# xuekt98/BBDM

Hardware: NVIDIA H100
Metric: denoising-steps/sec (UNet fwd) at 256^2 pixel-BBDM (higher is better)
Workload: dtype bf16x3 (split-bf16 tensor-core products, fp32 accumulate: fp32-class)

## Files before the change

bbdm_b200/csrc/conv_umma.cu:

```cuda
#include "tc_common.cuh"
#include <stdlib.h>

namespace bbdm {

constexpr int UM_BM = 128;
constexpr int UM_BK = 64;
constexpr int UM_THREADS = 384;
constexpr int UM_PRODUCER_REGS = 40, UM_CONSUMER_REGS = 232;
static_assert(128 * UM_PRODUCER_REGS + 256 * UM_CONSUMER_REGS <= 65536, "conv_umma: register split");
constexpr int UM_SLICES = 4;

struct ConvParams {
  int B, H, W, Cout;
  int TW, TH, TB, tiles_w, tiles_h, tiles_b, n_tiles;
  int kb_per_tap;
  int K1;
  int K2;
  int taps;
  int up2;
  int origin;
  int w_per_image;
  int kb_per_chunk;
  const float* bias; const float* bias2;
  const float* residual; int res_mode;
  float* out; __nv_bfloat16* out_hi; __nv_bfloat16* out_lo;
  int out_nchw_c;
  float* stats;
  unsigned long long* fault;
};

template <int BN>
struct UmmaCfg {
  static constexpr uint32_t A_BYTES = UM_BM * UM_BK * 2;
  static constexpr uint32_t W_BYTES = BN * UM_BK * 2;
  static constexpr uint32_t STAGE3 = 2 * A_BYTES + 2 * W_BYTES;
  static constexpr uint32_t STAGE1 = A_BYTES + W_BYTES;
  static constexpr uint32_t SMEM_BUDGET = 200 * 1024;
  static constexpr int STAGES3 = (SMEM_BUDGET / STAGE3) > 6 ? 6 : (SMEM_BUDGET / STAGE3);
  static constexpr int STAGES1 = (SMEM_BUDGET / STAGE1) > 8 ? 8 : (SMEM_BUDGET / STAGE1);
};

template <int BN, bool F16>
__device__ __forceinline__ void conv_mma(float* d, uint64_t da, uint64_t db) {
  if (F16) {
    if (BN == 128) wgmma_n128_f16<0>(d, da, db, 1u); else wgmma_n64_f16<0>(d, da, db, 1u);
  } else {
    if (BN == 128) wgmma_n128_bf16<0>(d, da, db, 1u); else wgmma_n64_bf16<0>(d, da, db, 1u);
  }
}

struct EpiTile {
  int nb, tw, th, tb, phase;
  int bb[2], hh[2], ww[2];
  bool valid[2];
  int64_t pix[2];
};

__device__ __forceinline__ EpiTile epi_tile(const ConvParams& p, int tile, int n_blocks, int warp, int lane) {
  EpiTile e;
  e.nb = tile % n_blocks;
  int mt = tile / n_blocks;
  e.phase = 0;
  if (p.up2) { e.phase = mt & 3; mt >>= 2; }
  e.tw = mt % p.tiles_w; mt /= p.tiles_w;
  e.th = mt % p.tiles_h;
  e.tb = mt / p.tiles_h;
  const int OH = p.up2 ? 2 * p.H : p.H, OW = p.up2 ? 2 * p.W : p.W;
#pragma unroll
  for (int ri = 0; ri < 2; ++ri) {
    const int row = 16 * warp + (lane >> 2) + 8 * ri;
    const int ws = e.tw * p.TW + row % p.TW;
    const int hs = e.th * p.TH + (row / p.TW) % p.TH;
    e.bb[ri] = e.tb * p.TB + row / (p.TW * p.TH);
    e.valid[ri] = ws < p.W && hs < p.H && e.bb[ri] < p.B;
    e.hh[ri] = p.up2 ? 2 * hs + (e.phase >> 1) : hs;
    e.ww[ri] = p.up2 ? 2 * ws + (e.phase & 1) : ws;
    e.pix[ri] = ((int64_t)e.bb[ri] * OH + e.hh[ri]) * OW + e.ww[ri];
  }
  return e;
}

template <int BN>
__device__ __forceinline__ void epi_slice(const ConvParams& p, const float* racc, EpiTile e, int s, int warp,
                                          int lane, float (*stats_s)[BN][2]) {
  constexpr int JS = BN / 8 / UM_SLICES;
  asm volatile("" : "+r"(e.nb), "+r"(e.bb[0]), "+r"(e.bb[1]), "+r"(e.hh[0]), "+r"(e.hh[1]), "+r"(e.ww[0]),
               "+r"(e.ww[1]), "+l"(e.pix[0]), "+l"(e.pix[1]));
  const int OH = p.up2 ? 2 * p.H : p.H, OW = p.up2 ? 2 * p.W : p.W;
  const int n0 = e.nb * BN + 2 * (lane & 3);
  float2 v[2][JS];
#pragma unroll
  for (int ri = 0; ri < 2; ++ri) {
#pragma unroll
    for (int j = 0; j < JS; ++j) {
      const int jj = JS * s + j;
      const int nc = n0 + 8 * jj;
      v[ri][j] = make_float2(racc[4 * jj + 2 * ri], racc[4 * jj + 2 * ri + 1]);
      if (p.bias) { const float2 b = *reinterpret_cast<const float2*>(p.bias + nc); v[ri][j].x += b.x; v[ri][j].y += b.y; }
      if (p.bias2) { const float2 b = *reinterpret_cast<const float2*>(p.bias2 + nc); v[ri][j].x += b.x; v[ri][j].y += b.y; }
    }
  }
  if (p.res_mode == BBDM_RES_SAME || p.res_mode == BBDM_RES_UP2) {
#pragma unroll
    for (int ri = 0; ri < 2; ++ri) {
      if (!e.valid[ri]) continue;
      const int64_t rpix = p.res_mode == BBDM_RES_SAME
                               ? e.pix[ri]
                               : ((int64_t)e.bb[ri] * (OH >> 1) + (e.hh[ri] >> 1)) * (OW >> 1) + (e.ww[ri] >> 1);
      const float* rp = p.residual + rpix * p.Cout + n0 + 8 * JS * s;
#pragma unroll
      for (int j = 0; j < JS; ++j) {
        const float2 t = *reinterpret_cast<const float2*>(rp + 8 * j);
        v[ri][j].x += t.x; v[ri][j].y += t.y;
      }
    }
  } else if (p.res_mode == BBDM_RES_DOWN2) {
    const int64_t W2 = (int64_t)OW * 2;
#pragma unroll
    for (int ri = 0; ri < 2; ++ri) {
      if (!e.valid[ri]) continue;
      const float* rp0 = p.residual + (((int64_t)e.bb[ri] * OH * 2 + e.hh[ri] * 2) * W2 + e.ww[ri] * 2) * p.Cout +
                         n0 + 8 * JS * s;
#pragma unroll
      for (int j = 0; j < JS; ++j) {
        const float* rp = rp0 + 8 * j;
        const float2 t0 = *reinterpret_cast<const float2*>(rp), t1 = *reinterpret_cast<const float2*>(rp + p.Cout);
        const float2 t2 = *reinterpret_cast<const float2*>(rp + W2 * p.Cout);
        const float2 t3 = *reinterpret_cast<const float2*>(rp + (W2 + 1) * p.Cout);
        v[ri][j].x += 0.25f * (((t0.x + t1.x) + t2.x) + t3.x);
        v[ri][j].y += 0.25f * (((t0.y + t1.y) + t2.y) + t3.y);
      }
    }
  }
  float ssum[2 * JS], ssq[2 * JS];
#pragma unroll
  for (int j = 0; j < 2 * JS; ++j) { ssum[j] = 0.f; ssq[j] = 0.f; }
#pragma unroll
  for (int ri = 0; ri < 2; ++ri) {
    if (!e.valid[ri]) continue;
    const int bb = e.bb[ri], hh = e.hh[ri], ww = e.ww[ri];
    const int64_t pix = e.pix[ri];
#pragma unroll
    for (int j = 0; j < JS; ++j) {
      const int nc = n0 + 8 * (JS * s + j);
      const float2 w = v[ri][j];
      if (p.out_nchw_c > 0) {
        if (nc < p.out_nchw_c) p.out[(((int64_t)bb * p.out_nchw_c + nc) * OH + hh) * OW + ww] = w.x;
        if (nc + 1 < p.out_nchw_c) p.out[(((int64_t)bb * p.out_nchw_c + nc + 1) * OH + hh) * OW + ww] = w.y;
      } else if (p.out) {
        *reinterpret_cast<float2*>(p.out + pix * p.Cout + nc) = w;
      }
      if (p.out_hi) {
        uint32_t h, l;
        split2x(w.x, w.y, h, l);
        *reinterpret_cast<uint32_t*>(p.out_hi + pix * p.Cout + nc) = h;
        *reinterpret_cast<uint32_t*>(p.out_lo + pix * p.Cout + nc) = l;
      }
      ssum[2 * j] += w.x; ssq[2 * j] += w.x * w.x;
      ssum[2 * j + 1] += w.y; ssq[2 * j + 1] += w.y * w.y;
    }
  }
  if (p.stats) {
#pragma unroll
    for (int j = 0; j < 2 * JS; ++j) {
#pragma unroll
      for (int off = 4; off < 32; off <<= 1) {
        ssum[j] += __shfl_xor_sync(0xffffffffu, ssum[j], off);
        ssq[j] += __shfl_xor_sync(0xffffffffu, ssq[j], off);
      }
    }
    if (lane < 4) {
#pragma unroll
      for (int j = 0; j < 2 * JS; ++j) {
        const int c = 8 * (JS * s + (j >> 1)) + 2 * lane + (j & 1);
        stats_s[warp][c][0] = ssum[j];
        stats_s[warp][c][1] = ssq[j];
      }
    }
  }
}

template <int BN>
__device__ __forceinline__ void epi_stats_out(const ConvParams& p, const EpiTile& e, float (*stats_s)[BN][2]) {
  if (!p.stats) return;
  asm volatile("bar.sync 1, 256;" ::: "memory");
  const int64_t tile_lin =
      (((int64_t)e.tb * p.tiles_w * p.tiles_h + e.th * p.tiles_w + e.tw) * (p.up2 ? 4 : 1) + e.phase) * 4;
  int i0 = threadIdx.x;
  asm volatile("" : "+r"(i0));
  for (int i = i0; i < 4 * BN; i += 256) {
    const int q = i / BN, c = i % BN;
    const float s = stats_s[2 * q][c][0] + stats_s[2 * q + 1][c][0];
    const float sq = stats_s[2 * q][c][1] + stats_s[2 * q + 1][c][1];
    *reinterpret_cast<float2*>(p.stats + ((tile_lin + q) * p.Cout + e.nb * BN + c) * 2) = make_float2(s, sq);
  }
  asm volatile("bar.sync 1, 256;" ::: "memory");
}

template <int BN>
__device__ __forceinline__ void epi_slices(const ConvParams& p, const float* racc, const EpiTile& e, int s_begin,
                                           int s_end, int warp, int lane, float (*stats_s)[BN][2]) {
#pragma unroll
  for (int s = 0; s < UM_SLICES; ++s)
    if (s >= s_begin && s < s_end) epi_slice<BN>(p, racc, e, s, warp, lane, stats_s);
}

template <int BN, int PASSES, bool F16>
__global__ void __launch_bounds__(UM_THREADS, 1)
conv_umma_kernel(const __grid_constant__ CUtensorMap map_a_hi, const __grid_constant__ CUtensorMap map_a_lo,
                 const __grid_constant__ CUtensorMap map_w_hi, const __grid_constant__ CUtensorMap map_w_lo,
                 const __grid_constant__ CUtensorMap map_a2_hi, const __grid_constant__ CUtensorMap map_a2_lo,
                 const __grid_constant__ CUtensorMap map_w2_hi, const __grid_constant__ CUtensorMap map_w2_lo,
                 const ConvParams p) {
  using Cfg = UmmaCfg<BN>;
  constexpr int STAGES = PASSES == 3 ? Cfg::STAGES3 : Cfg::STAGES1;
  constexpr uint32_t STAGE_BYTES = PASSES == 3 ? Cfg::STAGE3 : Cfg::STAGE1;
  constexpr uint32_t OFF_ALO = Cfg::A_BYTES;
  constexpr uint32_t OFF_WHI = PASSES == 3 ? 2 * Cfg::A_BYTES : Cfg::A_BYTES;
  constexpr uint32_t OFF_WLO = OFF_WHI + Cfg::W_BYTES;
  constexpr int NR = BN / 2;
  static_assert(STAGES >= 2, "need at least a double buffer");

  extern __shared__ uint8_t smem_raw[];
  __shared__ __align__(8) uint64_t bars[2 * 8];
  __shared__ int abort_s;
  __shared__ __align__(16) float stats_s[8][BN][2];

  const uint32_t tiles_base = (smem_u32(smem_raw) + 1023u) & ~1023u;
  const int warp = threadIdx.x >> 5, lane = threadIdx.x & 31;
  const uint32_t bar_full = smem_u32(&bars[0]);
  const uint32_t bar_empty = smem_u32(&bars[8]);
  volatile int* abort_flag = &abort_s;

  if (threadIdx.x == 0) {
    abort_s = 0;
    for (int i = 0; i < STAGES; ++i) { mbar_init(bar_full + 8 * i, 1); mbar_init(bar_empty + 8 * i, 8); }
    asm volatile("fence.mbarrier_init.release.cluster;" ::: "memory");
  }
  __syncthreads();

  const int n_blocks = p.Cout / BN;
  const int total_tiles = p.n_tiles * n_blocks * (p.up2 ? 4 : 1);
  const int KB = p.K1 + p.K2;

  if (warp >= 8) {
    setmaxnreg_dec<UM_PRODUCER_REGS>();
    if (warp == 8 && lane == 0) {
      int stage = 0;
      uint32_t phase_bit = 0;
      for (int tile = blockIdx.x; tile < total_tiles; tile += gridDim.x) {
        const int nb = tile % n_blocks;
        int mt = tile / n_blocks;
        int phase = 0;
        if (p.up2) { phase = mt & 3; mt >>= 2; }
        const int tw = mt % p.tiles_w; mt /= p.tiles_w;
        const int th = mt % p.tiles_h;
        const int tb = mt / p.tiles_h;
        const int w0 = tw * p.TW, h0 = th * p.TH, b0 = tb * p.TB, n0 = nb * BN;
        for (int kb = 0; kb < KB; ++kb) {
          mbar_wait(bar_empty + 8 * stage, phase_bit ^ 1, abort_flag, p.fault, 0xE0000000ull | (unsigned)kb);
          const uint32_t sbase = tiles_base + stage * STAGE_BYTES;
          const uint32_t full = bar_full + 8 * stage;
          mbar_expect_tx(full, STAGE_BYTES);
          if (kb < p.K1) {
            const int tap = kb / p.kb_per_tap, cb = kb - tap * p.kb_per_tap;
            int dy = 0, dx = 0, wtap = tap;
            if (p.up2) {
              const int r = tap >> 1, c = tap & 1;
              dy = (phase >> 1) ? r : r - 1;
              dx = (phase & 1) ? c : c - 1;
              wtap = phase * 4 + tap;
            } else if (p.taps == 9) { dy = tap / 3 - 1; dx = tap % 3 - 1; }
            else if (p.taps == 4) { dy = (tap >> 1) + p.origin; dx = (tap & 1) + p.origin; }
            else if (p.w_per_image) wtap = tb;
            tma_load_4d(sbase, &map_a_hi, full, cb * UM_BK, w0 + dx, h0 + dy, b0);
            if (PASSES == 3) tma_load_4d(sbase + OFF_ALO, &map_a_lo, full, cb * UM_BK, w0 + dx, h0 + dy, b0);
            tma_load_3d(sbase + OFF_WHI, &map_w_hi, full, cb * UM_BK, n0, wtap);
            if (PASSES == 3) tma_load_3d(sbase + OFF_WLO, &map_w_lo, full, cb * UM_BK, n0, wtap);
          } else {
            const int cb = kb - p.K1;
            tma_load_4d(sbase, &map_a2_hi, full, cb * UM_BK, w0, h0, b0);
            if (PASSES == 3) tma_load_4d(sbase + OFF_ALO, &map_a2_lo, full, cb * UM_BK, w0, h0, b0);
            tma_load_3d(sbase + OFF_WHI, &map_w2_hi, full, cb * UM_BK, n0, 0);
            if (PASSES == 3) tma_load_3d(sbase + OFF_WLO, &map_w2_lo, full, cb * UM_BK, n0, 0);
          }
          if (++stage == STAGES) { stage = 0; phase_bit ^= 1; }
        }
      }
    }
    return;
  }

  setmaxnreg_inc<UM_CONSUMER_REGS>();
  const int wg = warp >> 2;
  const uint32_t a_off = (uint32_t)wg * 64 * 128;
  int stage = 0;
  uint32_t phase_bit = 0;
  float racc[NR];
  EpiTile pend;
  bool pending = false;
  int slice = 0;
  for (int tile = blockIdx.x; tile < total_tiles; tile += gridDim.x) {
    for (int kb0 = 0; kb0 < KB; kb0 += p.kb_per_chunk) {
      const int kb1 = kb0 + p.kb_per_chunk < KB ? kb0 + p.kb_per_chunk : KB;
      float acc[NR];
#pragma unroll
      for (int j = 0; j < NR; ++j) acc[j] = 0.f;
      int prev = -1;
      for (int kb = kb0; kb < kb1; ++kb) {
        mbar_wait(bar_full + 8 * stage, phase_bit, abort_flag, p.fault, 0xF0000000ull | (unsigned)kb);
        const uint32_t sbase = tiles_base + stage * STAGE_BYTES;
        const uint64_t da_hi = make_sw128_desc(sbase + a_off);
        const uint64_t da_lo = make_sw128_desc(sbase + OFF_ALO + a_off);
        const uint64_t db_hi = make_sw128_desc(sbase + OFF_WHI);
        const uint64_t db_lo = make_sw128_desc(sbase + OFF_WLO);
        wgmma_fence();
#pragma unroll
        for (int k = 0; k < UM_BK / 16; ++k) {
          const uint64_t ko = (uint64_t)(k * 32 >> 4);
          if (PASSES == 3) {
            conv_mma<BN, F16>(acc, da_lo + ko, db_hi + ko);
            conv_mma<BN, F16>(acc, da_hi + ko, db_lo + ko);
          }
          conv_mma<BN, F16>(acc, da_hi + ko, db_hi + ko);
        }
        wgmma_commit();
        wgmma_wait<1>();
        if (prev >= 0 && lane == 0) mbar_arrive(bar_empty + 8 * prev);
        prev = stage;
        if (++stage == STAGES) { stage = 0; phase_bit ^= 1; }
        if (pending) {
          const int s_end = kb + 1 < kb1 ? slice + 1 : UM_SLICES;
          epi_slices<BN>(p, racc, pend, slice, s_end, warp, lane, stats_s);
          slice = s_end;
        }
      }
      if (pending) {
        epi_stats_out<BN>(p, pend, stats_s);
        pending = false;
      }
      wgmma_wait<0>();
      reg_fence<NR>(acc);
      if (lane == 0) mbar_arrive(bar_empty + 8 * prev);
      if (kb0 == 0) {
#pragma unroll
        for (int j = 0; j < NR; ++j) racc[j] = 0.f + acc[j];
      } else {
#pragma unroll
        for (int j = 0; j < NR; ++j) racc[j] += acc[j];
      }
    }
    pend = epi_tile(p, tile, n_blocks, warp, lane);
    pending = true;
    slice = 0;
  }
  if (pending) {
    epi_slices<BN>(p, racc, pend, 0, UM_SLICES, warp, lane, stats_s);
    epi_stats_out<BN>(p, pend, stats_s);
  }
}

static int make_act_map(CUtensorMap* m, const void* ptr, int B, int H, int W, int C, int TW, int TH, int TB,
                        bool f16) {
  EncodeTiledFn enc = get_encode();
  BBDM_REQUIRE(enc != nullptr, "cuTensorMapEncodeTiled entry point not available");
  cuuint64_t dims[4] = {(cuuint64_t)C, (cuuint64_t)W, (cuuint64_t)H, (cuuint64_t)B};
  cuuint64_t strides[3] = {(cuuint64_t)C * 2, (cuuint64_t)W * C * 2, (cuuint64_t)H * W * C * 2};
  cuuint32_t box[4] = {(cuuint32_t)UM_BK, (cuuint32_t)TW, (cuuint32_t)TH, (cuuint32_t)TB};
  cuuint32_t es[4] = {1, 1, 1, 1};
  CUresult r = enc(m, f16 ? CU_TENSOR_MAP_DATA_TYPE_FLOAT16 : CU_TENSOR_MAP_DATA_TYPE_BFLOAT16, 4, const_cast<void*>(ptr), dims, strides, box, es,
                   CU_TENSOR_MAP_INTERLEAVE_NONE, CU_TENSOR_MAP_SWIZZLE_128B, CU_TENSOR_MAP_L2_PROMOTION_L2_256B,
                   CU_TENSOR_MAP_FLOAT_OOB_FILL_NONE);
  BBDM_REQUIRE(r == CUDA_SUCCESS, "cuTensorMapEncodeTiled(activation) failed: %d (B=%d H=%d W=%d C=%d box=%dx%dx%d)",
               (int)r, B, H, W, C, TW, TH, TB);
  return BBDM_OK;
}

static int make_w_map(CUtensorMap* m, const void* ptr, int taps, int Cout, int Cin, int BN, bool f16) {
  EncodeTiledFn enc = get_encode();
  BBDM_REQUIRE(enc != nullptr, "cuTensorMapEncodeTiled entry point not available");
  cuuint64_t dims[3] = {(cuuint64_t)Cin, (cuuint64_t)Cout, (cuuint64_t)taps};
  cuuint64_t strides[2] = {(cuuint64_t)Cin * 2, (cuuint64_t)Cout * Cin * 2};
  cuuint32_t box[3] = {(cuuint32_t)UM_BK, (cuuint32_t)BN, 1};
  cuuint32_t es[3] = {1, 1, 1};
  CUresult r = enc(m, f16 ? CU_TENSOR_MAP_DATA_TYPE_FLOAT16 : CU_TENSOR_MAP_DATA_TYPE_BFLOAT16, 3, const_cast<void*>(ptr), dims, strides, box, es,
                   CU_TENSOR_MAP_INTERLEAVE_NONE, CU_TENSOR_MAP_SWIZZLE_128B, CU_TENSOR_MAP_L2_PROMOTION_L2_256B,
                   CU_TENSOR_MAP_FLOAT_OOB_FILL_NONE);
  BBDM_REQUIRE(r == CUDA_SUCCESS, "cuTensorMapEncodeTiled(weight) failed: %d (taps=%d Cout=%d Cin=%d BN=%d)", (int)r,
               taps, Cout, Cin, BN);
  return BBDM_OK;
}

static int pow2_floor(int x) { int p = 1; while (p * 2 <= x) p *= 2; return p; }
static int pow2_ceil(int x) { int p = 1; while (p < x) p *= 2; return p; }

template <int BN, int PASSES, bool F16>
static int launch_conv(const CUtensorMap* maps, const ConvParams& p, int grid, cudaStream_t s) {
  using Cfg = UmmaCfg<BN>;
  constexpr int STAGES = PASSES == 3 ? Cfg::STAGES3 : Cfg::STAGES1;
  constexpr uint32_t STAGE_BYTES = PASSES == 3 ? Cfg::STAGE3 : Cfg::STAGE1;
  const size_t smem = (size_t)STAGES * STAGE_BYTES + 1024;
  static DeviceOnce configured;
  if (configured.need()) {
    BBDM_CUDA_CHECK(cudaFuncSetAttribute(conv_umma_kernel<BN, PASSES, F16>, cudaFuncAttributeMaxDynamicSharedMemorySize, (int)smem));
    configured.mark();
  }
  conv_umma_kernel<BN, PASSES, F16><<<grid, UM_THREADS, smem, s>>>(maps[0], maps[1], maps[2], maps[3], maps[4], maps[5],
                                                                  maps[6], maps[7], p);
  BBDM_LAUNCH_CHECK();
  return BBDM_OK;
}

}

using namespace bbdm;

static void tile_geometry(int H, int W, int* TW, int* TH, int* TB) {
  *TW = pow2_floor(W) < 16 ? pow2_floor(W) : 16;
  const int th = pow2_ceil(H);
  *TH = th < UM_BM / *TW ? th : UM_BM / *TW;
  *TB = UM_BM / (*TW * *TH);
}

extern "C" int bbdm_conv_umma_geometry(int H, int W, int* TW, int* TH, int* TB, int* rows_per_image) {
  BBDM_REQUIRE(H > 0 && W >= 4, "conv_umma_geometry: need H > 0, W >= 4");
  int tw, th, tb;
  tile_geometry(H, W, &tw, &th, &tb);
  if (TW) *TW = tw;
  if (TH) *TH = th;
  if (TB) *TB = tb;
  if (rows_per_image) *rows_per_image = tb == 1 ? 4 * ((W + tw - 1) / tw) * ((H + th - 1) / th) : 0;
  return BBDM_OK;
}

extern "C" int bbdm_conv_umma(const BbdmConvArgs* a, void* stream) {
  BBDM_REQUIRE(a != nullptr, "conv_umma: null args");
  BBDM_REQUIRE(a->B > 0 && a->H > 0 && a->W > 0, "conv_umma: bad spatial shape");
  BBDM_REQUIRE(a->taps == 1 || a->taps == 9 || a->taps == 4, "conv_umma: taps must be 1, 4 or 9 (got %d)", a->taps);
  BBDM_REQUIRE(!a->upsample2x || (a->taps == 4 && a->Cin2 == 0), "conv_umma: upsample2x needs the 16 phase taps and no fused 1x1");
  BBDM_REQUIRE(a->Cin > 0 && a->Cin % 64 == 0, "conv_umma: Cin %% 64 != 0 (Cin=%d)", a->Cin);
  BBDM_REQUIRE(a->Cout > 0 && a->Cout % 64 == 0, "conv_umma: Cout %% 64 != 0 (Cout=%d)", a->Cout);
  BBDM_REQUIRE(a->Cin2 >= 0 && a->Cin2 % 64 == 0, "conv_umma: Cin2 %% 64 != 0 (Cin2=%d)", a->Cin2);
  BBDM_REQUIRE(a->passes == 1 || a->passes == 3, "conv_umma: passes must be 1 or 3");
  BBDM_REQUIRE(a->a_hi && a->w_hi && (a->passes == 1 || (a->a_lo && a->w_lo)), "conv_umma: missing operand plane");
  if (a->Cin2) BBDM_REQUIRE(a->a2_hi && a->w2_hi && (a->passes == 1 || (a->a2_lo && a->w2_lo)), "conv_umma: missing 1x1 operand plane");
  BBDM_REQUIRE(a->out || (a->out_hi && a->out_lo), "conv_umma: no output");
  BBDM_REQUIRE((a->out_hi == nullptr) == (a->out_lo == nullptr), "conv_umma: out hi/lo must come in pairs");
  BBDM_REQUIRE(a->res_mode >= 0 && a->res_mode <= 3 && (a->res_mode == 0 || a->residual), "conv_umma: bad residual");
  if (a->res_mode == BBDM_RES_UP2 && !a->upsample2x) BBDM_REQUIRE(a->H % 2 == 0 && a->W % 2 == 0, "conv_umma: RES_UP2 needs even H, W");
  BBDM_REQUIRE(a->W >= 4, "conv_umma: W < 4 not supported (use conv_direct)");
  BBDM_REQUIRE(a->window_origin == 0 || a->window_origin == -1, "conv_umma: window_origin must be 0 or -1 (got %d)",
               a->window_origin);
  BBDM_REQUIRE(a->window_origin == 0 || (a->taps == 4 && !a->upsample2x),
               "conv_umma: window_origin -1 needs taps == 4 and no upsample2x");
  const bool wpi = a->weights_per_image != 0, f16 = a->operand_f16 != 0;
  if (wpi) BBDM_REQUIRE(a->taps == 1 && a->Cin2 == 0 && !a->upsample2x, "conv_umma: weights_per_image needs taps == 1 and no fused operand");

  ConvParams p;
  p.B = a->B; p.H = a->H; p.W = a->W; p.Cout = a->Cout;
  tile_geometry(a->H, a->W, &p.TW, &p.TH, &p.TB);
  p.tiles_w = (a->W + p.TW - 1) / p.TW;
  p.tiles_h = (a->H + p.TH - 1) / p.TH;
  p.tiles_b = (a->B + p.TB - 1) / p.TB;
  p.n_tiles = p.tiles_w * p.tiles_h * p.tiles_b;
  int BN = (a->Cout % 128 == 0) ? 128 : 64;
  {
    const int64_t m_tiles = (int64_t)p.n_tiles * (a->upsample2x ? 4 : 1);
    const int64_t want = (int64_t)(0.7 * num_sms());
    if (BN > 64 && m_tiles * (a->Cout / BN) < want) BN = 64;
  }
  p.kb_per_tap = a->Cin / UM_BK;
  p.K1 = a->taps * p.kb_per_tap;
  p.K2 = a->Cin2 / UM_BK;
  p.taps = a->taps;
  p.up2 = a->upsample2x ? 1 : 0;
  p.origin = a->window_origin;
  p.w_per_image = wpi ? 1 : 0;
  static int wino_chunk = -1;
  if (wino_chunk < 0) { const char* e = getenv("BBDM_WINO_CHUNK"); wino_chunk = (e && atoi(e) > 0) ? atoi(e) : 0; }
  const int wchunk = wino_chunk ? wino_chunk : (a->Cin >= 512 ? 4 : 2);
  p.kb_per_chunk = wpi ? wchunk : (a->passes == 3 ? 4 : 8);
  if (wpi) BBDM_REQUIRE(p.TB == 1, "conv_umma: weights_per_image needs 128-pixel tiles inside one image (H*W >= 128)");
  p.bias = a->bias; p.bias2 = a->Cin2 ? a->bias2 : nullptr;
  p.residual = a->residual; p.res_mode = a->res_mode;
  p.out = a->out; p.out_hi = (__nv_bfloat16*)a->out_hi; p.out_lo = (__nv_bfloat16*)a->out_lo;
  p.out_nchw_c = a->out_nchw_channels;
  p.stats = a->stats_partial;
  BBDM_REQUIRE(p.out_nchw_c >= 0 && p.out_nchw_c <= a->Cout && (p.out_nchw_c == 0 || (a->out && !a->out_hi)),
               "conv_umma: bad out_nchw_channels");
  p.fault = device_fault_ptr();
  BBDM_REQUIRE(p.fault != nullptr, "conv_umma: device fault word unavailable");

  BBDM_REQUIRE(p.stats == nullptr || (p.TB == 1 && p.out_nchw_c == 0),
               "conv_umma: stats_partial needs a tile inside one image (H*W >= 128) and NHWC output");
  CUtensorMap maps[8];
  int rc;
  if ((rc = make_act_map(&maps[0], a->a_hi, a->B, a->H, a->W, a->Cin, p.TW, p.TH, p.TB, f16))) return rc;
  if ((rc = make_act_map(&maps[1], a->passes == 3 ? a->a_lo : a->a_hi, a->B, a->H, a->W, a->Cin, p.TW, p.TH, p.TB, f16))) return rc;
  const int wtaps = a->upsample2x ? 16 : (wpi ? a->B : a->taps);
  if ((rc = make_w_map(&maps[2], a->w_hi, wtaps, a->Cout, a->Cin, BN, f16))) return rc;
  if ((rc = make_w_map(&maps[3], a->passes == 3 ? a->w_lo : a->w_hi, wtaps, a->Cout, a->Cin, BN, f16))) return rc;
  if (a->Cin2) {
    if ((rc = make_act_map(&maps[4], a->a2_hi, a->B, a->H, a->W, a->Cin2, p.TW, p.TH, p.TB, f16))) return rc;
    if ((rc = make_act_map(&maps[5], a->passes == 3 ? a->a2_lo : a->a2_hi, a->B, a->H, a->W, a->Cin2, p.TW, p.TH, p.TB, f16))) return rc;
    if ((rc = make_w_map(&maps[6], a->w2_hi, 1, a->Cout, a->Cin2, BN, f16))) return rc;
    if ((rc = make_w_map(&maps[7], a->passes == 3 ? a->w2_lo : a->w2_hi, 1, a->Cout, a->Cin2, BN, f16))) return rc;
  } else {
    maps[4] = maps[0]; maps[5] = maps[1]; maps[6] = maps[2]; maps[7] = maps[3];
  }
  const int64_t total = (int64_t)p.n_tiles * (a->Cout / BN) * (p.up2 ? 4 : 1);
  BBDM_REQUIRE(total < (1ll << 30), "conv_umma: too many tiles");
  const int grid = (int)(total < num_sms() ? total : num_sms());
  cudaStream_t s = (cudaStream_t)stream;
  const bool p3 = a->passes == 3;
  if (BN == 128) {
    if (f16) return p3 ? launch_conv<128, 3, true>(maps, p, grid, s) : launch_conv<128, 1, true>(maps, p, grid, s);
    return p3 ? launch_conv<128, 3, false>(maps, p, grid, s) : launch_conv<128, 1, false>(maps, p, grid, s);
  }
  if (f16) return p3 ? launch_conv<64, 3, true>(maps, p, grid, s) : launch_conv<64, 1, true>(maps, p, grid, s);
  return p3 ? launch_conv<64, 3, false>(maps, p, grid, s) : launch_conv<64, 1, false>(maps, p, grid, s);
}
```

bbdm_b200/csrc/tc_common.cuh:

```cuda
#pragma once
#include "common.cuh"
#include <cuda.h>

namespace bbdm {

__device__ __forceinline__ uint32_t smem_u32(const void* p) {
  return (uint32_t)__cvta_generic_to_shared(p);
}
__device__ __forceinline__ void mbar_init(uint32_t bar, uint32_t count) {
  asm volatile("mbarrier.init.shared::cta.b64 [%0], %1;" ::"r"(bar), "r"(count));
}
__device__ __forceinline__ void mbar_expect_tx(uint32_t bar, uint32_t bytes) {
  asm volatile("mbarrier.arrive.expect_tx.shared::cta.b64 _, [%0], %1;" ::"r"(bar), "r"(bytes) : "memory");
}
__device__ __forceinline__ void mbar_arrive(uint32_t bar) {
  asm volatile("mbarrier.arrive.shared::cta.b64 _, [%0];" ::"r"(bar) : "memory");
}
__device__ __forceinline__ bool mbar_try_wait(uint32_t bar, uint32_t parity) {
  uint32_t ok;
  asm volatile(
      "{\n\t.reg .pred P;\n\t"
      "mbarrier.try_wait.parity.shared::cta.b64 P, [%1], %2;\n\t"
      "selp.u32 %0, 1, 0, P;\n\t}"
      : "=r"(ok) : "r"(bar), "r"(parity) : "memory");
  return ok != 0;
}
__device__ __forceinline__ void mbar_wait(uint32_t bar, uint32_t parity, volatile int* abort_flag,
                                          unsigned long long* fault, unsigned long long code) {
  if (mbar_try_wait(bar, parity)) return;
  const long long t0 = clock64();
  while (!mbar_try_wait(bar, parity)) {
    if (*abort_flag) return;
    if (clock64() - t0 > 1000000000ll) {
      *abort_flag = 1;
      atomicExch(fault, code);
      return;
    }
  }
}
__device__ __forceinline__ void tma_load_4d(uint32_t dst, const CUtensorMap* map, uint32_t bar,
                                            int c0, int c1, int c2, int c3) {
  asm volatile(
      "cp.async.bulk.tensor.4d.shared::cluster.global.mbarrier::complete_tx::bytes"
      " [%0], [%1, {%3, %4, %5, %6}], [%2];"
      ::"r"(dst), "l"(map), "r"(bar), "r"(c0), "r"(c1), "r"(c2), "r"(c3) : "memory");
}
__device__ __forceinline__ void tma_load_4d_im2col(uint32_t dst, const CUtensorMap* map, uint32_t bar,
                                                   int c0, int w, int h, int n, uint16_t off_w, uint16_t off_h) {
  asm volatile(
      "cp.async.bulk.tensor.4d.shared::cluster.global.im2col.mbarrier::complete_tx::bytes"
      " [%0], [%1, {%3, %4, %5, %6}], [%2], {%7, %8};"
      ::"r"(dst), "l"(map), "r"(bar), "r"(c0), "r"(w), "r"(h), "r"(n), "h"(off_w), "h"(off_h) : "memory");
}
__device__ __forceinline__ void tma_load_2d(uint32_t dst, const CUtensorMap* map, uint32_t bar, int c0, int c1) {
  asm volatile(
      "cp.async.bulk.tensor.2d.shared::cluster.global.mbarrier::complete_tx::bytes"
      " [%0], [%1, {%3, %4}], [%2];"
      ::"r"(dst), "l"(map), "r"(bar), "r"(c0), "r"(c1) : "memory");
}
__device__ __forceinline__ void tma_load_3d(uint32_t dst, const CUtensorMap* map, uint32_t bar,
                                            int c0, int c1, int c2) {
  asm volatile(
      "cp.async.bulk.tensor.3d.shared::cluster.global.mbarrier::complete_tx::bytes"
      " [%0], [%1, {%3, %4, %5}], [%2];"
      ::"r"(dst), "l"(map), "r"(bar), "r"(c0), "r"(c1), "r"(c2) : "memory");
}
__device__ __forceinline__ void wgmma_fence() { asm volatile("wgmma.fence.sync.aligned;" ::: "memory"); }
__device__ __forceinline__ void wgmma_commit() { asm volatile("wgmma.commit_group.sync.aligned;" ::: "memory"); }
template <int N>
__device__ __forceinline__ void wgmma_wait() { asm volatile("wgmma.wait_group.sync.aligned %0;" ::"n"(N) : "memory"); }
template <int R>
__device__ __forceinline__ void reg_fence(float* d) {
#pragma unroll
  for (int i = 0; i < R; ++i) asm volatile("" : "+f"(d[i])::"memory");
}

__device__ __forceinline__ uint64_t make_sw128_desc(uint32_t saddr, uint32_t lbo = 16) {
  uint64_t d = 0;
  d |= (uint64_t)((saddr & 0x3FFFF) >> 4);
  d |= (uint64_t)((lbo & 0x3FFFF) >> 4) << 16;
  d |= (uint64_t)(1024 >> 4) << 32;
  d |= (uint64_t)1 << 62;
  return d;
}

template <int TB>
__device__ __forceinline__ void wgmma_n64_bf16(float* d, uint64_t da, uint64_t db, uint32_t scale_d) {
  asm volatile(
      "{\n\t.reg .pred p;\n\tsetp.ne.b32 p, %34, 0;\n\t"
      "wgmma.mma_async.sync.aligned.m64n64k16.f32.bf16.bf16 "
      "{%0, %1, %2, %3, %4, %5, %6, %7, %8, %9, %10, %11, %12, %13, %14, %15, %16, %17, %18, %19, %20, %21, %22, %23, %24, %25, %26, %27, %28, %29, %30, %31}, %32, %33, p, 1, 1, 0, %35;\n\t}"
      : "+f"(d[0]), "+f"(d[1]), "+f"(d[2]), "+f"(d[3]), "+f"(d[4]), "+f"(d[5]), "+f"(d[6]), "+f"(d[7]), "+f"(d[8]), "+f"(d[9]), "+f"(d[10]), "+f"(d[11]), "+f"(d[12]), "+f"(d[13]), "+f"(d[14]), "+f"(d[15]), "+f"(d[16]), "+f"(d[17]), "+f"(d[18]), "+f"(d[19]), "+f"(d[20]), "+f"(d[21]), "+f"(d[22]), "+f"(d[23]), "+f"(d[24]), "+f"(d[25]), "+f"(d[26]), "+f"(d[27]), "+f"(d[28]), "+f"(d[29]), "+f"(d[30]), "+f"(d[31])
      : "l"(da), "l"(db), "r"(scale_d), "n"(TB));
}
template <int TB>
__device__ __forceinline__ void wgmma_n64_f16(float* d, uint64_t da, uint64_t db, uint32_t scale_d) {
  asm volatile(
      "{\n\t.reg .pred p;\n\tsetp.ne.b32 p, %34, 0;\n\t"
      "wgmma.mma_async.sync.aligned.m64n64k16.f32.f16.f16 "
      "{%0, %1, %2, %3, %4, %5, %6, %7, %8, %9, %10, %11, %12, %13, %14, %15, %16, %17, %18, %19, %20, %21, %22, %23, %24, %25, %26, %27, %28, %29, %30, %31}, %32, %33, p, 1, 1, 0, %35;\n\t}"
      : "+f"(d[0]), "+f"(d[1]), "+f"(d[2]), "+f"(d[3]), "+f"(d[4]), "+f"(d[5]), "+f"(d[6]), "+f"(d[7]), "+f"(d[8]), "+f"(d[9]), "+f"(d[10]), "+f"(d[11]), "+f"(d[12]), "+f"(d[13]), "+f"(d[14]), "+f"(d[15]), "+f"(d[16]), "+f"(d[17]), "+f"(d[18]), "+f"(d[19]), "+f"(d[20]), "+f"(d[21]), "+f"(d[22]), "+f"(d[23]), "+f"(d[24]), "+f"(d[25]), "+f"(d[26]), "+f"(d[27]), "+f"(d[28]), "+f"(d[29]), "+f"(d[30]), "+f"(d[31])
      : "l"(da), "l"(db), "r"(scale_d), "n"(TB));
}
template <int TB>
__device__ __forceinline__ void wgmma_n128_bf16(float* d, uint64_t da, uint64_t db, uint32_t scale_d) {
  asm volatile(
      "{\n\t.reg .pred p;\n\tsetp.ne.b32 p, %66, 0;\n\t"
      "wgmma.mma_async.sync.aligned.m64n128k16.f32.bf16.bf16 "
      "{%0, %1, %2, %3, %4, %5, %6, %7, %8, %9, %10, %11, %12, %13, %14, %15, %16, %17, %18, %19, %20, %21, %22, %23, %24, %25, %26, %27, %28, %29, %30, %31, %32, %33, %34, %35, %36, %37, %38, %39, %40, %41, %42, %43, %44, %45, %46, %47, %48, %49, %50, %51, %52, %53, %54, %55, %56, %57, %58, %59, %60, %61, %62, %63}, %64, %65, p, 1, 1, 0, %67;\n\t}"
      : "+f"(d[0]), "+f"(d[1]), "+f"(d[2]), "+f"(d[3]), "+f"(d[4]), "+f"(d[5]), "+f"(d[6]), "+f"(d[7]), "+f"(d[8]), "+f"(d[9]), "+f"(d[10]), "+f"(d[11]), "+f"(d[12]), "+f"(d[13]), "+f"(d[14]), "+f"(d[15]), "+f"(d[16]), "+f"(d[17]), "+f"(d[18]), "+f"(d[19]), "+f"(d[20]), "+f"(d[21]), "+f"(d[22]), "+f"(d[23]), "+f"(d[24]), "+f"(d[25]), "+f"(d[26]), "+f"(d[27]), "+f"(d[28]), "+f"(d[29]), "+f"(d[30]), "+f"(d[31]), "+f"(d[32]), "+f"(d[33]), "+f"(d[34]), "+f"(d[35]), "+f"(d[36]), "+f"(d[37]), "+f"(d[38]), "+f"(d[39]), "+f"(d[40]), "+f"(d[41]), "+f"(d[42]), "+f"(d[43]), "+f"(d[44]), "+f"(d[45]), "+f"(d[46]), "+f"(d[47]), "+f"(d[48]), "+f"(d[49]), "+f"(d[50]), "+f"(d[51]), "+f"(d[52]), "+f"(d[53]), "+f"(d[54]), "+f"(d[55]), "+f"(d[56]), "+f"(d[57]), "+f"(d[58]), "+f"(d[59]), "+f"(d[60]), "+f"(d[61]), "+f"(d[62]), "+f"(d[63])
      : "l"(da), "l"(db), "r"(scale_d), "n"(TB));
}
template <int TB>
__device__ __forceinline__ void wgmma_n128_f16(float* d, uint64_t da, uint64_t db, uint32_t scale_d) {
  asm volatile(
      "{\n\t.reg .pred p;\n\tsetp.ne.b32 p, %66, 0;\n\t"
      "wgmma.mma_async.sync.aligned.m64n128k16.f32.f16.f16 "
      "{%0, %1, %2, %3, %4, %5, %6, %7, %8, %9, %10, %11, %12, %13, %14, %15, %16, %17, %18, %19, %20, %21, %22, %23, %24, %25, %26, %27, %28, %29, %30, %31, %32, %33, %34, %35, %36, %37, %38, %39, %40, %41, %42, %43, %44, %45, %46, %47, %48, %49, %50, %51, %52, %53, %54, %55, %56, %57, %58, %59, %60, %61, %62, %63}, %64, %65, p, 1, 1, 0, %67;\n\t}"
      : "+f"(d[0]), "+f"(d[1]), "+f"(d[2]), "+f"(d[3]), "+f"(d[4]), "+f"(d[5]), "+f"(d[6]), "+f"(d[7]), "+f"(d[8]), "+f"(d[9]), "+f"(d[10]), "+f"(d[11]), "+f"(d[12]), "+f"(d[13]), "+f"(d[14]), "+f"(d[15]), "+f"(d[16]), "+f"(d[17]), "+f"(d[18]), "+f"(d[19]), "+f"(d[20]), "+f"(d[21]), "+f"(d[22]), "+f"(d[23]), "+f"(d[24]), "+f"(d[25]), "+f"(d[26]), "+f"(d[27]), "+f"(d[28]), "+f"(d[29]), "+f"(d[30]), "+f"(d[31]), "+f"(d[32]), "+f"(d[33]), "+f"(d[34]), "+f"(d[35]), "+f"(d[36]), "+f"(d[37]), "+f"(d[38]), "+f"(d[39]), "+f"(d[40]), "+f"(d[41]), "+f"(d[42]), "+f"(d[43]), "+f"(d[44]), "+f"(d[45]), "+f"(d[46]), "+f"(d[47]), "+f"(d[48]), "+f"(d[49]), "+f"(d[50]), "+f"(d[51]), "+f"(d[52]), "+f"(d[53]), "+f"(d[54]), "+f"(d[55]), "+f"(d[56]), "+f"(d[57]), "+f"(d[58]), "+f"(d[59]), "+f"(d[60]), "+f"(d[61]), "+f"(d[62]), "+f"(d[63])
      : "l"(da), "l"(db), "r"(scale_d), "n"(TB));
}
template <int TB>
__device__ __forceinline__ void wgmma_rs_n64_bf16(float* d, const uint32_t* a, uint64_t db, uint32_t scale_d) {
  asm volatile(
      "{\n\t.reg .pred p;\n\tsetp.ne.b32 p, %37, 0;\n\t"
      "wgmma.mma_async.sync.aligned.m64n64k16.f32.bf16.bf16 "
      "{%0, %1, %2, %3, %4, %5, %6, %7, %8, %9, %10, %11, %12, %13, %14, %15, %16, %17, %18, %19, %20, %21, %22, %23, %24, %25, %26, %27, %28, %29, %30, %31}, {%32, %33, %34, %35}, %36, p, 1, 1, %38;\n\t}"
      : "+f"(d[0]), "+f"(d[1]), "+f"(d[2]), "+f"(d[3]), "+f"(d[4]), "+f"(d[5]), "+f"(d[6]), "+f"(d[7]), "+f"(d[8]), "+f"(d[9]), "+f"(d[10]), "+f"(d[11]), "+f"(d[12]), "+f"(d[13]), "+f"(d[14]), "+f"(d[15]), "+f"(d[16]), "+f"(d[17]), "+f"(d[18]), "+f"(d[19]), "+f"(d[20]), "+f"(d[21]), "+f"(d[22]), "+f"(d[23]), "+f"(d[24]), "+f"(d[25]), "+f"(d[26]), "+f"(d[27]), "+f"(d[28]), "+f"(d[29]), "+f"(d[30]), "+f"(d[31])
      : "r"(a[0]), "r"(a[1]), "r"(a[2]), "r"(a[3]), "l"(db), "r"(scale_d), "n"(TB));
}

template <int N>
__device__ __forceinline__ void setmaxnreg_inc() { asm volatile("setmaxnreg.inc.sync.aligned.u32 %0;" ::"n"(N)); }
template <int N>
__device__ __forceinline__ void setmaxnreg_dec() { asm volatile("setmaxnreg.dec.sync.aligned.u32 %0;" ::"n"(N)); }

__device__ __forceinline__ float ex2_approx(float x) {
  float y;
  asm("ex2.approx.ftz.f32 %0, %1;" : "=f"(y) : "f"(x));
  return y;
}
__device__ __forceinline__ void st_shared_v4(uint32_t addr, uint32_t a, uint32_t b, uint32_t c, uint32_t d) {
  asm volatile("st.shared.v4.b32 [%0], {%1, %2, %3, %4};" ::"r"(addr), "r"(a), "r"(b), "r"(c), "r"(d) : "memory");
}

typedef CUresult (*EncodeTiledFn)(CUtensorMap*, CUtensorMapDataType, cuuint32_t, void*, const cuuint64_t*,
                                  const cuuint64_t*, const cuuint32_t*, const cuuint32_t*, CUtensorMapInterleave,
                                  CUtensorMapSwizzle, CUtensorMapL2promotion, CUtensorMapFloatOOBfill);

static inline EncodeTiledFn get_encode() {
  static EncodeTiledFn fn = nullptr;
  if (!fn) {
    void* p = nullptr;
    cudaDriverEntryPointQueryResult qres;
    if (cudaGetDriverEntryPoint("cuTensorMapEncodeTiled", &p, cudaEnableDefault, &qres) == cudaSuccess &&
        qres == cudaDriverEntryPointSuccess)
      fn = (EncodeTiledFn)p;
  }
  return fn;
}

typedef CUresult (*EncodeIm2colFn)(CUtensorMap*, CUtensorMapDataType, cuuint32_t, void*, const cuuint64_t*,
                                   const cuuint64_t*, const int*, const int*, cuuint32_t, cuuint32_t, const cuuint32_t*,
                                   CUtensorMapInterleave, CUtensorMapSwizzle, CUtensorMapL2promotion,
                                   CUtensorMapFloatOOBfill);

static inline EncodeIm2colFn get_encode_im2col() {
  static EncodeIm2colFn fn = nullptr;
  if (!fn) {
    void* p = nullptr;
    cudaDriverEntryPointQueryResult qres;
    if (cudaGetDriverEntryPoint("cuTensorMapEncodeIm2col", &p, cudaEnableDefault, &qres) == cudaSuccess &&
        qres == cudaDriverEntryPointSuccess)
      fn = (EncodeIm2colFn)p;
  }
  return fn;
}

}
```

Before: 6.061.

## Reuse one halo activation box across all nine conv taps

For 3x3 convolutions without a fused second operand or upsampling, the producer now loads a single (TW+2)x(TH+2) halo box of activations per channel block into a double-buffered region. The consumer then forms the nine tap operands by offsetting the shared-memory wgmma descriptor with a custom stride-byte offset, while the weights stream through their own ring. This removes the repeated per-tap TMA loads of overlapping activation tiles and frees ring space for more weight stages. In exchange it adds a second barrier pipeline and fixes the tile shape to 8x16. It also relies on descriptor offsets that are not 1024-byte aligned working with the 128-byte swizzle layout.

```diff
diff --git a/bbdm_b200/csrc/conv_umma.cu b/bbdm_b200/csrc/conv_umma.cu
--- a/bbdm_b200/csrc/conv_umma.cu
+++ b/bbdm_b200/csrc/conv_umma.cu
@@ -40,6 +40,18 @@
   static constexpr int STAGES1 = (SMEM_BUDGET / STAGE1) > 8 ? 8 : (SMEM_BUDGET / STAGE1);
 };
 
+constexpr int HALO_TW = 8, HALO_TH = 16, HALO_PITCH = HALO_TW + 2, HALO_ROWS = HALO_TH + 2;
+template <int BN, int PASSES>
+struct HaloCfg {
+  static constexpr uint32_t BOX_BYTES = HALO_PITCH * HALO_ROWS * 128;
+  static constexpr uint32_t PLANE = (BOX_BYTES + 1023u) & ~1023u;
+  static constexpr uint32_t A_BUF = PASSES == 3 ? 2 * PLANE : PLANE;
+  static constexpr uint32_t W_STAGE = PASSES == 3 ? 2 * UmmaCfg<BN>::W_BYTES : UmmaCfg<BN>::W_BYTES;
+  static constexpr uint32_t W_ROOM = UmmaCfg<BN>::SMEM_BUDGET - 2 * A_BUF;
+  static constexpr int STAGES = (W_ROOM / W_STAGE) > 8 ? 8 : (W_ROOM / W_STAGE);
+  static constexpr uint32_t SMEM = 2 * A_BUF + STAGES * W_STAGE;
+};
+
 template <int BN, bool F16>
 __device__ __forceinline__ void conv_mma(float* d, uint64_t da, uint64_t db) {
   if (F16) {
@@ -205,7 +217,7 @@
     if (s >= s_begin && s < s_end) epi_slice<BN>(p, racc, e, s, warp, lane, stats_s);
 }
 
-template <int BN, int PASSES, bool F16>
+template <int BN, int PASSES, bool F16, bool HALO>
 __global__ void __launch_bounds__(UM_THREADS, 1)
 conv_umma_kernel(const __grid_constant__ CUtensorMap map_a_hi, const __grid_constant__ CUtensorMap map_a_lo,
                  const __grid_constant__ CUtensorMap map_w_hi, const __grid_constant__ CUtensorMap map_w_lo,
@@ -213,16 +225,17 @@
                  const __grid_constant__ CUtensorMap map_w2_hi, const __grid_constant__ CUtensorMap map_w2_lo,
                  const ConvParams p) {
   using Cfg = UmmaCfg<BN>;
-  constexpr int STAGES = PASSES == 3 ? Cfg::STAGES3 : Cfg::STAGES1;
-  constexpr uint32_t STAGE_BYTES = PASSES == 3 ? Cfg::STAGE3 : Cfg::STAGE1;
+  using HCfg = HaloCfg<BN, PASSES>;
+  constexpr int STAGES = HALO ? HCfg::STAGES : PASSES == 3 ? Cfg::STAGES3 : Cfg::STAGES1;
+  constexpr uint32_t STAGE_BYTES = HALO ? HCfg::W_STAGE : PASSES == 3 ? Cfg::STAGE3 : Cfg::STAGE1;
   constexpr uint32_t OFF_ALO = Cfg::A_BYTES;
-  constexpr uint32_t OFF_WHI = PASSES == 3 ? 2 * Cfg::A_BYTES : Cfg::A_BYTES;
+  constexpr uint32_t OFF_WHI = HALO ? 0 : PASSES == 3 ? 2 * Cfg::A_BYTES : Cfg::A_BYTES;
   constexpr uint32_t OFF_WLO = OFF_WHI + Cfg::W_BYTES;
   constexpr int NR = BN / 2;
-  static_assert(STAGES >= 2, "need at least a double buffer");
+  static_assert(STAGES >= 2 && STAGES <= 8, "need at least a double buffer, at most 8 barriers");
 
   extern __shared__ uint8_t smem_raw[];
-  __shared__ __align__(8) uint64_t bars[2 * 8];
+  __shared__ __align__(8) uint64_t bars[2 * 8 + 4];
   __shared__ int abort_s;
   __shared__ __align__(16) float stats_s[8][BN][2];
 
@@ -230,11 +243,16 @@
   const int warp = threadIdx.x >> 5, lane = threadIdx.x & 31;
   const uint32_t bar_full = smem_u32(&bars[0]);
   const uint32_t bar_empty = smem_u32(&bars[8]);
+  const uint32_t bar_afull = smem_u32(&bars[16]);
+  const uint32_t bar_aempty = smem_u32(&bars[18]);
+  const uint32_t ring_base = HALO ? tiles_base + 2 * HCfg::A_BUF : tiles_base;
   volatile int* abort_flag = &abort_s;
 
   if (threadIdx.x == 0) {
     abort_s = 0;
     for (int i = 0; i < STAGES; ++i) { mbar_init(bar_full + 8 * i, 1); mbar_init(bar_empty + 8 * i, 8); }
+    if (HALO)
+      for (int i = 0; i < 2; ++i) { mbar_init(bar_afull + 8 * i, 1); mbar_init(bar_aempty + 8 * i, 8); }
     asm volatile("fence.mbarrier_init.release.cluster;" ::: "memory");
   }
   __syncthreads();
@@ -245,7 +263,40 @@
 
   if (warp >= 8) {
     setmaxnreg_dec<UM_PRODUCER_REGS>();
-    if (warp == 8 && lane == 0) {
+    if (HALO && warp == 8 && lane == 0) {
+      int stage = 0, abuf = 0;
+      uint32_t phase_bit = 0, aphase = 0;
+      auto issue_box = [&](int tile, int cb) {
+        const int mt = tile / n_blocks;
+        const int w0 = (mt % p.tiles_w) * HALO_TW, h0 = (mt / p.tiles_w % p.tiles_h) * HALO_TH;
+        const int b0 = mt / (p.tiles_w * p.tiles_h);
+        mbar_wait(bar_aempty + 8 * abuf, aphase ^ 1, abort_flag, p.fault, 0xE8000000ull | (unsigned)cb);
+        const uint32_t dst = tiles_base + abuf * HCfg::A_BUF, full = bar_afull + 8 * abuf;
+        mbar_expect_tx(full, (PASSES == 3 ? 2 : 1) * HCfg::BOX_BYTES);
+        tma_load_4d(dst, &map_a_hi, full, cb * UM_BK, w0 - 1, h0 - 1, b0);
+        if (PASSES == 3) tma_load_4d(dst + HCfg::PLANE, &map_a_lo, full, cb * UM_BK, w0 - 1, h0 - 1, b0);
+        if (++abuf == 2) { abuf = 0; aphase ^= 1; }
+      };
+      if ((int)blockIdx.x < total_tiles) issue_box(blockIdx.x, 0);
+      for (int tile = blockIdx.x; tile < total_tiles; tile += gridDim.x) {
+        const int n0 = (tile % n_blocks) * BN;
+        for (int cb = 0; cb < p.kb_per_tap; ++cb) {
+          for (int tap = 0; tap < 9; ++tap) {
+            mbar_wait(bar_empty + 8 * stage, phase_bit ^ 1, abort_flag, p.fault, 0xE0000000ull | (unsigned)(cb * 9 + tap));
+            const uint32_t sbase = ring_base + stage * STAGE_BYTES;
+            const uint32_t full = bar_full + 8 * stage;
+            mbar_expect_tx(full, STAGE_BYTES);
+            tma_load_3d(sbase + OFF_WHI, &map_w_hi, full, cb * UM_BK, n0, tap);
+            if (PASSES == 3) tma_load_3d(sbase + OFF_WLO, &map_w_lo, full, cb * UM_BK, n0, tap);
+            if (++stage == STAGES) { stage = 0; phase_bit ^= 1; }
+            if (tap == 3) {
+              if (cb + 1 < p.kb_per_tap) issue_box(tile, cb + 1);
+              else if (tile + (int)gridDim.x < total_tiles) issue_box(tile + gridDim.x, 0);
+            }
+          }
+        }
+      }
+    } else if (!HALO && warp == 8 && lane == 0) {
       int stage = 0;
       uint32_t phase_bit = 0;
       for (int tile = blockIdx.x; tile < total_tiles; tile += gridDim.x) {
@@ -294,24 +345,36 @@
   setmaxnreg_inc<UM_CONSUMER_REGS>();
   const int wg = warp >> 2;
   const uint32_t a_off = (uint32_t)wg * 64 * 128;
-  int stage = 0;
-  uint32_t phase_bit = 0;
+  int stage = 0, abuf = 0;
+  uint32_t phase_bit = 0, aphase = 0;
   float racc[NR];
   EpiTile pend;
   bool pending = false;
   int slice = 0;
   for (int tile = blockIdx.x; tile < total_tiles; tile += gridDim.x) {
+    int tap = 0;
     for (int kb0 = 0; kb0 < KB; kb0 += p.kb_per_chunk) {
       const int kb1 = kb0 + p.kb_per_chunk < KB ? kb0 + p.kb_per_chunk : KB;
       float acc[NR];
 #pragma unroll
       for (int j = 0; j < NR; ++j) acc[j] = 0.f;
-      int prev = -1;
+      int prev = -1, prev_a = -1;
       for (int kb = kb0; kb < kb1; ++kb) {
+        if (HALO && tap == 0)
+          mbar_wait(bar_afull + 8 * abuf, aphase, abort_flag, p.fault, 0xF8000000ull | (unsigned)kb);
         mbar_wait(bar_full + 8 * stage, phase_bit, abort_flag, p.fault, 0xF0000000ull | (unsigned)kb);
-        const uint32_t sbase = tiles_base + stage * STAGE_BYTES;
-        const uint64_t da_hi = make_sw128_desc(sbase + a_off);
-        const uint64_t da_lo = make_sw128_desc(sbase + OFF_ALO + a_off);
+        const uint32_t sbase = ring_base + stage * STAGE_BYTES;
+        uint64_t da_hi, da_lo;
+        if (HALO) {
+          const uint32_t abase = tiles_base + abuf * HCfg::A_BUF;
+          const int ky = tap >= 6 ? 2 : tap >= 3 ? 1 : 0, kx = tap - 3 * ky;
+          const uint32_t off = (uint32_t)(((8 * wg + ky) * HALO_PITCH + kx) * 128);
+          da_hi = make_sw128_desc(abase + off, 16, HALO_PITCH * 128);
+          da_lo = make_sw128_desc(abase + HCfg::PLANE + off, 16, HALO_PITCH * 128);
+        } else {
+          da_hi = make_sw128_desc(sbase + a_off);
+          da_lo = make_sw128_desc(sbase + OFF_ALO + a_off);
+        }
         const uint64_t db_hi = make_sw128_desc(sbase + OFF_WHI);
         const uint64_t db_lo = make_sw128_desc(sbase + OFF_WLO);
         wgmma_fence();
@@ -327,8 +390,14 @@
         wgmma_commit();
         wgmma_wait<1>();
         if (prev >= 0 && lane == 0) mbar_arrive(bar_empty + 8 * prev);
+        if (HALO && prev_a >= 0 && lane == 0) mbar_arrive(bar_aempty + 8 * prev_a);
         prev = stage;
         if (++stage == STAGES) { stage = 0; phase_bit ^= 1; }
+        if (HALO) {
+          prev_a = tap == 8 ? abuf : -1;
+          if (tap == 8 && ++abuf == 2) { abuf = 0; aphase ^= 1; }
+          tap = tap < 8 ? tap + 1 : 0;
+        }
         if (pending) {
           const int s_end = kb + 1 < kb1 ? slice + 1 : UM_SLICES;
           epi_slices<BN>(p, racc, pend, slice, s_end, warp, lane, stats_s);
@@ -342,6 +411,7 @@
       wgmma_wait<0>();
       reg_fence<NR>(acc);
       if (lane == 0) mbar_arrive(bar_empty + 8 * prev);
+      if (HALO && prev_a >= 0 && lane == 0) mbar_arrive(bar_aempty + 8 * prev_a);
       if (kb0 == 0) {
 #pragma unroll
         for (int j = 0; j < NR; ++j) racc[j] = 0.f + acc[j];
@@ -394,19 +464,19 @@
 static int pow2_floor(int x) { int p = 1; while (p * 2 <= x) p *= 2; return p; }
 static int pow2_ceil(int x) { int p = 1; while (p < x) p *= 2; return p; }
 
-template <int BN, int PASSES, bool F16>
+template <int BN, int PASSES, bool F16, bool HALO>
 static int launch_conv(const CUtensorMap* maps, const ConvParams& p, int grid, cudaStream_t s) {
   using Cfg = UmmaCfg<BN>;
   constexpr int STAGES = PASSES == 3 ? Cfg::STAGES3 : Cfg::STAGES1;
   constexpr uint32_t STAGE_BYTES = PASSES == 3 ? Cfg::STAGE3 : Cfg::STAGE1;
-  const size_t smem = (size_t)STAGES * STAGE_BYTES + 1024;
+  const size_t smem = (HALO ? (size_t)HaloCfg<BN, PASSES>::SMEM : (size_t)STAGES * STAGE_BYTES) + 1024;
   static DeviceOnce configured;
   if (configured.need()) {
-    BBDM_CUDA_CHECK(cudaFuncSetAttribute(conv_umma_kernel<BN, PASSES, F16>, cudaFuncAttributeMaxDynamicSharedMemorySize, (int)smem));
+    BBDM_CUDA_CHECK(cudaFuncSetAttribute(conv_umma_kernel<BN, PASSES, F16, HALO>, cudaFuncAttributeMaxDynamicSharedMemorySize, (int)smem));
     configured.mark();
   }
-  conv_umma_kernel<BN, PASSES, F16><<<grid, UM_THREADS, smem, s>>>(maps[0], maps[1], maps[2], maps[3], maps[4], maps[5],
-                                                                  maps[6], maps[7], p);
+  conv_umma_kernel<BN, PASSES, F16, HALO><<<grid, UM_THREADS, smem, s>>>(maps[0], maps[1], maps[2], maps[3], maps[4],
+                                                                        maps[5], maps[6], maps[7], p);
   BBDM_LAUNCH_CHECK();
   return BBDM_OK;
 }
@@ -414,6 +484,16 @@
 }
 
 using namespace bbdm;
+
+template <bool HALO>
+static int launch_form(const CUtensorMap* maps, const ConvParams& p, int grid, cudaStream_t s, int BN, bool p3, bool f16) {
+  if (BN == 128) {
+    if (f16) return p3 ? launch_conv<128, 3, true, HALO>(maps, p, grid, s) : launch_conv<128, 1, true, HALO>(maps, p, grid, s);
+    return p3 ? launch_conv<128, 3, false, HALO>(maps, p, grid, s) : launch_conv<128, 1, false, HALO>(maps, p, grid, s);
+  }
+  if (f16) return p3 ? launch_conv<64, 3, true, HALO>(maps, p, grid, s) : launch_conv<64, 1, true, HALO>(maps, p, grid, s);
+  return p3 ? launch_conv<64, 3, false, HALO>(maps, p, grid, s) : launch_conv<64, 1, false, HALO>(maps, p, grid, s);
+}
 
 static void tile_geometry(int H, int W, int* TW, int* TH, int* TB) {
   *TW = pow2_floor(W) < 16 ? pow2_floor(W) : 16;
@@ -456,9 +536,17 @@
   const bool wpi = a->weights_per_image != 0, f16 = a->operand_f16 != 0;
   if (wpi) BBDM_REQUIRE(a->taps == 1 && a->Cin2 == 0 && !a->upsample2x, "conv_umma: weights_per_image needs taps == 1 and no fused operand");
 
+  static int halo_env = -1;
+  if (halo_env < 0) { const char* e = getenv("BBDM_CONV_HALO"); halo_env = (e && atoi(e) == 0) ? 0 : 1; }
   ConvParams p;
   p.B = a->B; p.H = a->H; p.W = a->W; p.Cout = a->Cout;
   tile_geometry(a->H, a->W, &p.TW, &p.TH, &p.TB);
+  const bool halo = halo_env && a->taps == 9 && a->Cin2 == 0 && !a->upsample2x && !wpi && a->W >= HALO_TW &&
+                    a->H >= HALO_TH &&
+                    (a->stats_partial == nullptr ||
+                     (p.TB == 1 && ((a->W + p.TW - 1) / p.TW) * ((a->H + p.TH - 1) / p.TH) ==
+                                       ((a->W + HALO_TW - 1) / HALO_TW) * ((a->H + HALO_TH - 1) / HALO_TH)));
+  if (halo) { p.TW = HALO_TW; p.TH = HALO_TH; p.TB = 1; }
   p.tiles_w = (a->W + p.TW - 1) / p.TW;
   p.tiles_h = (a->H + p.TH - 1) / p.TH;
   p.tiles_b = (a->B + p.TB - 1) / p.TB;
@@ -495,8 +583,9 @@
                "conv_umma: stats_partial needs a tile inside one image (H*W >= 128) and NHWC output");
   CUtensorMap maps[8];
   int rc;
-  if ((rc = make_act_map(&maps[0], a->a_hi, a->B, a->H, a->W, a->Cin, p.TW, p.TH, p.TB, f16))) return rc;
-  if ((rc = make_act_map(&maps[1], a->passes == 3 ? a->a_lo : a->a_hi, a->B, a->H, a->W, a->Cin, p.TW, p.TH, p.TB, f16))) return rc;
+  const int atw = halo ? HALO_PITCH : p.TW, ath = halo ? HALO_ROWS : p.TH;
+  if ((rc = make_act_map(&maps[0], a->a_hi, a->B, a->H, a->W, a->Cin, atw, ath, p.TB, f16))) return rc;
+  if ((rc = make_act_map(&maps[1], a->passes == 3 ? a->a_lo : a->a_hi, a->B, a->H, a->W, a->Cin, atw, ath, p.TB, f16))) return rc;
   const int wtaps = a->upsample2x ? 16 : (wpi ? a->B : a->taps);
   if ((rc = make_w_map(&maps[2], a->w_hi, wtaps, a->Cout, a->Cin, BN, f16))) return rc;
   if ((rc = make_w_map(&maps[3], a->passes == 3 ? a->w_lo : a->w_hi, wtaps, a->Cout, a->Cin, BN, f16))) return rc;
@@ -512,11 +601,6 @@
   BBDM_REQUIRE(total < (1ll << 30), "conv_umma: too many tiles");
   const int grid = (int)(total < num_sms() ? total : num_sms());
   cudaStream_t s = (cudaStream_t)stream;
-  const bool p3 = a->passes == 3;
-  if (BN == 128) {
-    if (f16) return p3 ? launch_conv<128, 3, true>(maps, p, grid, s) : launch_conv<128, 1, true>(maps, p, grid, s);
-    return p3 ? launch_conv<128, 3, false>(maps, p, grid, s) : launch_conv<128, 1, false>(maps, p, grid, s);
-  }
-  if (f16) return p3 ? launch_conv<64, 3, true>(maps, p, grid, s) : launch_conv<64, 1, true>(maps, p, grid, s);
-  return p3 ? launch_conv<64, 3, false>(maps, p, grid, s) : launch_conv<64, 1, false>(maps, p, grid, s);
-}
+  if (halo) return launch_form<true>(maps, p, grid, s, BN, a->passes == 3, f16);
+  return launch_form<false>(maps, p, grid, s, BN, a->passes == 3, f16);
+}
diff --git a/bbdm_b200/csrc/tc_common.cuh b/bbdm_b200/csrc/tc_common.cuh
--- a/bbdm_b200/csrc/tc_common.cuh
+++ b/bbdm_b200/csrc/tc_common.cuh
@@ -75,11 +75,11 @@
   for (int i = 0; i < R; ++i) asm volatile("" : "+f"(d[i])::"memory");
 }
 
-__device__ __forceinline__ uint64_t make_sw128_desc(uint32_t saddr, uint32_t lbo = 16) {
+__device__ __forceinline__ uint64_t make_sw128_desc(uint32_t saddr, uint32_t lbo = 16, uint32_t sbo = 1024) {
   uint64_t d = 0;
   d |= (uint64_t)((saddr & 0x3FFFF) >> 4);
   d |= (uint64_t)((lbo & 0x3FFFF) >> 4) << 16;
-  d |= (uint64_t)(1024 >> 4) << 32;
+  d |= (uint64_t)((sbo & 0x3FFFF) >> 4) << 32;
   d |= (uint64_t)1 << 62;
   return d;
 }
```

After: 6.076, median of 6. About the same (+0.2%).
